# mcmilk/7-Zip-zstd

Measured on NVIDIA H100. Metric: zstd-L3 encode+decode throughput, higher is better.
Workload: dtype u8

## Files before the change

### 7-zip-zstd_b200/csrc/zstd_enc_entropy.cu

```cuda
#include "b2z_device.cuh"
#include "b2z_kernels.h"

namespace b2z {

__device__ const uint32_t d_LL_base[36] = { 0,1,2,3,4,5,6,7,8,9,10,11,12,13,14,15,
    16,18,20,22,24,28,32,40,48,64,0x80,0x100,0x200,0x400,0x800,0x1000,0x2000,0x4000,0x8000,0x10000 };
__device__ const uint8_t d_LL_bits[36] = { 0,0,0,0,0,0,0,0,0,0,0,0,0,0,0,0,
    1,1,1,1,2,2,3,3,4,6,7,8,9,10,11,12,13,14,15,16 };
__device__ const uint32_t d_ML_base[53] = { 3,4,5,6,7,8,9,10,11,12,13,14,15,16,17,18,
    19,20,21,22,23,24,25,26,27,28,29,30,31,32,33,34,
    35,37,39,41,43,47,51,59,67,83,99,0x83,0x103,0x203,0x403,0x803,0x1003,0x2003,0x4003,0x8003,0x10003 };
__device__ const uint8_t d_ML_bits[53] = { 0,0,0,0,0,0,0,0,0,0,0,0,0,0,0,0,
    0,0,0,0,0,0,0,0,0,0,0,0,0,0,0,0,
    1,1,1,1,2,2,3,3,4,4,5,7,8,9,10,11,12,13,14,15,16 };
__device__ const int16_t d_LL_defNorm[36] = { 4,3,2,2,2,2,2,2,2,2,2,2,2,1,1,1,
    2,2,2,2,2,2,2,2,2,3,2,1,1,1,1,1,-1,-1,-1,-1 };
__device__ const int16_t d_ML_defNorm[53] = { 1,4,3,2,2,2,2,2,2,1,1,1,1,1,1,1,
    1,1,1,1,1,1,1,1,1,1,1,1,1,1,1,1,
    1,1,1,1,1,1,1,1,1,1,1,1,1,1,-1,-1,-1,-1,-1,-1,-1 };
__device__ const int16_t d_OF_defNorm[29] = { 1,1,1,1,1,1,2,2,2,1,1,1,1,1,1,1,
    1,1,1,1,1,1,1,1,-1,-1,-1,-1,-1 };
__device__ const uint8_t d_log2frac[32] = { 0, 11, 22, 33, 43, 53, 63, 72, 82, 91, 100, 108, 116, 125, 132, 140,
    148, 155, 162, 169, 176, 182, 189, 195, 201, 207, 213, 219, 225, 230, 236, 241 };

__device__ __forceinline__ uint32_t ll_code(uint32_t ll) {
    if (ll < 16) return ll;
    if (ll < 24) return 16 + ((ll - 16) >> 1);
    if (ll < 32) return 20 + ((ll - 24) >> 2);
    if (ll < 48) return 22 + ((ll - 32) >> 3);
    if (ll < 64) return 24;
    return highbit32(ll) + 19;
}
__device__ __forceinline__ uint32_t ml_code(uint32_t m) {
    if (m < 32) return m;
    if (m < 40) return 32 + ((m - 32) >> 1);
    if (m < 48) return 36 + ((m - 40) >> 2);
    if (m < 64) return 38 + ((m - 48) >> 3);
    if (m < 96) return 40 + ((m - 64) >> 4);
    if (m < 128) return 42;
    return highbit32(m) + 36;
}

__device__ __forceinline__ uint32_t warp_sum(uint32_t v) {
    for (int d = 16; d; d >>= 1) v += __shfl_xor_sync(B2Z_FULL, v, d);
    return v;
}
__device__ __forceinline__ uint32_t warp_max(uint32_t v) {
    for (int d = 16; d; d >>= 1) { const uint32_t o = __shfl_xor_sync(B2Z_FULL, v, d); v = o > v ? o : v; }
    return v;
}

struct FseCT {
    uint16_t state[512];
    int32_t  dfs[64];
    uint32_t dnb[64];
    uint32_t log;
};

#define STAGE_WORDS 384
#define STAGE_FLUSH_BITS (STAGE_WORDS * 32 - 3072)

struct WarpWS {
    uint32_t hist[256];
    uint16_t hufCode[256];
    uint8_t  hufLen[256];
    union {
        struct { uint32_t w[512]; uint16_t parent[512]; uint8_t order[256]; uint8_t depth[512]; uint32_t key[256]; } hb;
        struct { FseCT ct[3]; } fse;
    } u;
    uint8_t  spread[512];
    int16_t  norm[64];
    uint16_t cumul[66];
    uint16_t cpos[66];
    uint32_t rk[16], rstart[16], rnext[16];
    uint32_t wcnt[16];
    uint32_t stage[STAGE_WORDS];
};

#define ENT_ST_OF 512u
#define ENT_ST_ML 768u
#define ENT_ST_N  1280u
#define ENT_SY_OF 36u
#define ENT_SY_ML 68u
#define ENT_SY_N  121u
struct EntTables {
    uint16_t state[ENT_ST_N];
    uint2    sym[ENT_SY_N];
    uint32_t pad[2];
};
struct EntRec {
    uint32_t run;
    uint32_t bodyHead;
    uint32_t logs;
    uint32_t pad0;
    uint16_t fin[4];
    uint32_t pad1[2];
    EntTables tab;
};
static_assert(sizeof(EntTables) % 16 == 0 && sizeof(EntRec) % 16 == 0 && offsetof(EntRec, tab) % 16 == 0, "EntRec is copied in 16-byte units");
#define ENT_SCRATCH_STRIDE ((size_t)sizeof(EntRec) + (size_t)B2Z_MAXSEQ * 4u)
static_assert(sizeof(EntRec) + (size_t)B2Z_MAXSEQ * 4u <= (size_t)B2Z_BLOCK * 4u, "stage E scratch must fit the block's candidate words");

struct BitW {
    uint8_t* p; uint64_t acc; uint32_t nb;
    __device__ __forceinline__ void init(uint8_t* q) { p = q; acc = 0; nb = 0; }
    __device__ __forceinline__ void add(uint32_t v, uint32_t n) {
        acc |= (uint64_t)(v & (n >= 32 ? 0xFFFFFFFFu : ((1u << n) - 1u))) << nb; nb += n;
        while (nb >= 8) { *p++ = (uint8_t)acc; acc >>= 8; nb -= 8; }
    }
    __device__ __forceinline__ uint8_t* close() { add(1, 1); if (nb) { *p++ = (uint8_t)acc; acc = 0; nb = 0; } return p; }
    __device__ __forceinline__ uint8_t* flush_partial() { if (nb) { *p++ = (uint8_t)acc; acc = 0; nb = 0; } return p; }
};

__device__ void fse_build_ctable(WarpWS* ws, FseCT* ct, const int16_t* norm, uint32_t maxSym, uint32_t log, uint32_t lane) {
    const uint32_t size = 1u << log, mask = size - 1u, step = (size >> 1) + (size >> 3) + 3u, lt = (1u << lane) - 1u;
    uint16_t* cumul = ws->cumul; uint16_t* cpos = ws->cpos; uint8_t* spread = ws->spread;
    uint32_t cu = 0, cp = 0, nLow = 0;
    for (uint32_t s0 = 0; s0 <= maxSym; s0 += 32) {
        const uint32_t s = s0 + lane;
        const int n = s <= maxSym ? norm[s] : 0;
        uint32_t tc, tp;
        const uint32_t ec = warp_excl_scan(n == -1 ? 1u : (n > 0 ? (uint32_t)n : 0u), lane, &tc);
        const uint32_t ep = warp_excl_scan(n > 0 ? (uint32_t)n : 0u, lane, &tp);
        const uint32_t low = __ballot_sync(B2Z_FULL, n == -1);
// ... 200 lines not shown
    maxW = warp_max(maxW);
    if (lane < 16) ws->wcnt[lane] = 0;
    __syncwarp();
    uint32_t fseSize = 0;
    if (nw > 1) {
        for (uint32_t s = lane; s < nw; s += 32) atomicAdd(&ws->wcnt[wt[s]], 1u);
        __syncwarp();
        const uint32_t maxCnt = warp_max(lane <= maxW ? ws->wcnt[lane] : 0u);
        if (maxCnt != nw && maxCnt > 1) {
            uint32_t log = 6;
            const uint32_t minBits = highbit32(nw) + 1u, symBits = highbit32(maxW + 1u) + 2u;
            const uint32_t lo = minBits < symBits ? minBits : symBits;
            const uint32_t want = highbit32(nw - 1u) >= 2u ? highbit32(nw - 1u) - 2u : 0u;
            if (want < log) log = want;
            if (log < lo) log = lo;
            if (log < 5) log = 5;
            if (log > 6) log = 6;
            int16_t* norm = ws->norm;
            fse_normalize(norm, log, ws->wcnt, nw, maxW, lane);
            uint8_t* tmp = dst + 1;
            uint32_t hs = 0;
            if (lane == 0) hs = fse_write_ncount(tmp, norm, maxW, log);
            hs = __shfl_sync(B2Z_FULL, hs, 0);
            FseCT* ct = reinterpret_cast<FseCT*>(ws->u.hb.w);
            fse_build_ctable(ws, ct, norm, maxW, log, lane);
            if (lane == 0) {
                BitW b; b.init(tmp + hs);
                uint32_t i = nw, s1, s2, nb, bits;
                if (nw & 1u) { s1 = fse_init_state(ct, wt[--i]); s2 = fse_init_state(ct, wt[--i]);
                               bits = fse_encode(ct, &s1, wt[--i], &nb); b.add(bits, nb); }
                else { s2 = fse_init_state(ct, wt[--i]); s1 = fse_init_state(ct, wt[--i]); }
                while (i > 0) {
                    bits = fse_encode(ct, &s2, wt[--i], &nb); b.add(bits, nb);
                    bits = fse_encode(ct, &s1, wt[--i], &nb); b.add(bits, nb);
                }
                b.add(s2, log); b.add(s1, log);
                fseSize = (uint32_t)(b.close() - tmp);
            }
            fseSize = __shfl_sync(B2Z_FULL, fseSize, 0);
        }
    }
    const uint32_t rawSize = (nw + 1u) / 2u;
    if (fseSize && fseSize < 128u && (fseSize < rawSize || nw > 128u)) { if (lane == 0) dst[0] = (uint8_t)fseSize; return 1u + fseSize; }
    if (nw > 128u || nw == 0u) return 0;
    if (lane == 0) dst[0] = (uint8_t)(127u + nw);
    for (uint32_t i = 2u * lane; i < nw; i += 64) dst[1 + i / 2] = (uint8_t)((wt[i] << 4) | (i + 1 < nw ? wt[i + 1] : 0));
    return 1u + rawSize;
}
static_assert(sizeof(FseCT) <= sizeof(uint32_t) * 512, "weights FseCT must fit in hb.w");

struct Stager {
    uint32_t* stage; uint8_t* out; uint32_t bits;
    __device__ __forceinline__ void init(uint32_t* s, uint8_t* o, uint32_t lane) {
        stage = s; out = o; bits = 0;
        for (uint32_t i = lane; i < STAGE_WORDS; i += 32) stage[i] = 0;
        __syncwarp();
    }
    __device__ __forceinline__ void put(uint32_t off, uint64_t lo, uint32_t hi, uint32_t nb) {
        if (!nb) return;
        const uint32_t wi = off >> 5, sh = off & 31u;
        const uint32_t w0 = (uint32_t)lo, w1 = (uint32_t)(lo >> 32);
        atomicOr(&stage[wi], w0 << sh);
        const uint32_t end = sh + nb;
        if (end > 32) atomicOr(&stage[wi + 1], sh ? (uint32_t)((((uint64_t)w1 << 32) | w0) >> (32 - sh)) : w1);
        if (end > 64) atomicOr(&stage[wi + 2], sh ? (uint32_t)((((uint64_t)hi << 32) | w1) >> (32 - sh)) : hi);
        if (end > 96) atomicOr(&stage[wi + 3], sh ? (hi >> (32 - sh)) : 0u);
    }
    __device__ __forceinline__ void flush(uint32_t lane, bool force) {
        __syncwarp();
        const uint32_t nbytes = force ? (bits + 7u) >> 3 : bits >> 3;
        const uint8_t* sb = reinterpret_cast<const uint8_t*>(stage);
        for (uint32_t i = lane; i < nbytes; i += 32) out[i] = sb[i];
        const uint32_t rem = force ? 0u : (bits & 7u);
        const uint32_t carry = rem ? sb[nbytes] : 0u;
        __syncwarp();
        for (uint32_t i = lane; i < STAGE_WORDS; i += 32) stage[i] = (i == 0) ? carry : 0u;
        __syncwarp();
        out += nbytes; bits = rem;
    }
};

__device__ uint32_t huf_encode_stream(WarpWS* ws, Stager& st, const uint8_t* __restrict__ lit, uint32_t a, uint32_t b, uint32_t lane) {
    uint8_t* start = st.out;
    for (uint32_t hi = b; hi > a;) {
        const uint32_t cnt = (hi - a) < 128u ? (hi - a) : 128u;
        uint64_t code = 0; uint32_t nb = 0;
#pragma unroll
        for (uint32_t j = 0; j < 4; j++) {
            const uint32_t k = lane * 4u + j;
            if (k < cnt) { const uint32_t s = lit[hi - 1u - k]; code |= (uint64_t)ws->hufCode[s] << nb; nb += ws->hufLen[s]; }
        }
        uint32_t total; const uint32_t off = warp_excl_scan(nb, lane, &total);
        st.put(st.bits + off, code, 0, nb);
        st.bits += total; hi -= cnt;
        if (st.bits > STAGE_FLUSH_BITS) st.flush(lane, false);
    }
    if (lane == 0) st.put(st.bits, 1, 0, 1);
    st.bits += 1;
    st.flush(lane, true);
    return (uint32_t)(st.out - start);
}

__device__ __forceinline__ void warp_copy(uint8_t* dst, const uint8_t* __restrict__ src, uint32_t n, uint32_t lane) {
    for (uint32_t i = lane; i < n; i += 32) dst[i] = src[i];
}

__device__ uint32_t choose_seq_table(WarpWS* ws, FseCT* ct, uint8_t* dst, const uint32_t* count, uint32_t nbSeq, uint32_t maxSymAll,
                                     uint32_t maxLog, const int16_t* defNorm, uint32_t defMaxSym, uint32_t defLog, uint32_t* mode, uint32_t lane) {
    uint32_t maxSym = 0, present = 0, big = 0;
    for (uint32_t s = lane; s <= maxSymAll; s += 32) if (count[s]) { maxSym = s; present++; if (count[s] > big) big = count[s]; }
    maxSym = warp_max(maxSym); present = warp_sum(present); big = warp_max(big);
    if (big == nbSeq && !(nbSeq <= 2 && maxSym <= defMaxSym)) {
        for (uint32_t s = lane; s < 64; s += 32) { ct->dnb[s] = 0; ct->dfs[s] = 0; }
        if (lane < 2) ct->state[lane] = 0;
        if (lane == 0) { ct->log = 0; dst[0] = (uint8_t)maxSym; }
        __syncwarp();
        *mode = 1; return 1;
    }
    int16_t* norm = ws->norm;
    uint64_t costDef = ~0ull;
    if (maxSym <= defMaxSym) {
        for (uint32_t s = lane; s <= defMaxSym; s += 32) norm[s] = defNorm[s];
        __syncwarp();
        costDef = fse_cost_fx8(count, norm, maxSym, defLog, lane);
        __syncwarp();
    }
    const uint32_t hbN = highbit32(nbSeq > 1 ? nbSeq - 1u : 1u);
    uint32_t log = hbN >= 2 ? hbN - 2u : 0u;
    const uint32_t minA = highbit32(nbSeq) + 1u, minB = highbit32(maxSym ? maxSym : 1u) + 2u, lo = minA < minB ? minA : minB;
    if (log > maxLog) log = maxLog;
    if (log < lo) log = lo;
    if (log < 5) log = 5;
    if (log > maxLog) log = maxLog;
    while ((1u << log) < present) log++;
    fse_normalize(norm, log, count, nbSeq, maxSym, lane);
    uint32_t hs = 0;
    if (lane == 0) hs = fse_write_ncount(dst, norm, maxSym, log);
    hs = __shfl_sync(B2Z_FULL, hs, 0);
    const uint64_t costFse = fse_cost_fx8(count, norm, maxSym, log, lane) + ((uint64_t)hs << 11);
    __syncwarp();
    if (costDef <= costFse || big == nbSeq) {
        for (uint32_t s = lane; s <= defMaxSym; s += 32) norm[s] = defNorm[s];
        __syncwarp();
        fse_build_ctable(ws, ct, norm, defMaxSym, defLog, lane); *mode = 0; return 0;
    }
    fse_build_ctable(ws, ct, norm, maxSym, log, lane); *mode = 2; return hs;
}

struct BlockGeom { uint32_t blkSize, last; size_t litOff; };
__device__ __forceinline__ BlockGeom block_geom(const EncGeom& g, uint64_t srcSize, uint32_t blk) {
    const uint32_t blocksPerFrame = 1u << (g.frameLog - 17u);
    const uint64_t frame = blk / blocksPerFrame; const uint32_t bif = blk % blocksPerFrame;
    const uint64_t f0 = frame << g.frameLog;
    const uint64_t fn = enc_frame_bytes(g, srcSize, frame);
    const uint64_t b0 = (uint64_t)bif << 17;
    BlockGeom r;
    r.blkSize = (uint32_t)((fn - b0) < B2Z_BLOCK ? (fn - b0) : B2Z_BLOCK);
    r.last = (b0 + r.blkSize == fn) ? 1u : 0u;
    r.litOff = (size_t)(f0 + b0);
    return r;
}
__device__ __forceinline__ void put_hdr3(uint8_t* out, uint32_t h) { out[0] = (uint8_t)h; out[1] = (uint8_t)(h >> 8); out[2] = (uint8_t)(h >> 16); }

__device__ uint32_t finish_block(uint8_t* out, const uint8_t* __restrict__ bsrc, uint32_t blkSize, uint32_t last, uint32_t bodySize, bool overCap, uint32_t lane) {
    if (!overCap && bodySize < blkSize) {
        if (lane == 0) put_hdr3(out, last | (2u << 1) | (bodySize << 3));
        return 3 + bodySize;
    }
    __syncwarp();
    if (lane == 0) put_hdr3(out, last | (blkSize << 3));
    warp_copy(out + 3, bsrc, blkSize, lane);
    return 3 + blkSize;
}

__global__ void __launch_bounds__(B2Z_ENT_WARPS * 32)
zstd_enc_tables_kernel(const uint8_t* __restrict__ src, uint64_t srcSize, EncGeom g,
                       const uint64_t* __restrict__ seqs, const uint32_t* __restrict__ nseqArr,
                       const uint8_t* __restrict__ lits, const uint32_t* __restrict__ nlitArr,
                       uint8_t* __restrict__ slots, uint32_t* __restrict__ slotSize, uint8_t* __restrict__ scratch, uint32_t nBlocks) {
    __shared__ WarpWS wsAll[B2Z_ENT_WARPS];
    const uint32_t lane = threadIdx.x & 31u, wib = threadIdx.x >> 5;
    WarpWS* ws = &wsAll[wib];
    for (uint32_t blk = blockIdx.x * B2Z_ENT_WARPS + wib; blk < nBlocks; blk += gridDim.x * B2Z_ENT_WARPS) {
        const BlockGeom bg = block_geom(g, srcSize, blk);
        const uint32_t blkSize = bg.blkSize, last = bg.last;
        const uint8_t* bsrc = src + bg.litOff;
        const uint8_t* lit = lits + bg.litOff;
        const uint64_t* sq = seqs + (size_t)blk * B2Z_MAXSEQ;
        const uint32_t nbSeq = nseqArr[blk], nlit = nlitArr[blk];
        uint8_t* out = slots + (size_t)blk * B2Z_SLOT;
        uint8_t* body = out + 3;
        EntRec* rec = reinterpret_cast<EntRec*>(scratch + (size_t)blk * ENT_SCRATCH_STRIDE);

        bool rle = false;
        if (blkSize > 1 && nbSeq == 1 && nlit == 1) {
            const uint64_t s0 = sq[0];
            rle = B2Z_SEQ_LL(s0) == 1 && B2Z_SEQ_ML(s0) == blkSize - 1u && B2Z_SEQ_OFFBASE(s0) == 4u;
        }
        if (rle) {
            if (lane == 0) { put_hdr3(out, last | (1u << 1) | (blkSize << 3)); out[3] = bsrc[0]; slotSize[blk] = 4; rec->run = 0; }
            continue;
        }

        for (uint32_t i = lane; i < 256; i += 32) ws->hist[i] = 0;
        __syncwarp();
        for (uint32_t i = lane * 4; i < nlit; i += 128) {
            const uint32_t v = *reinterpret_cast<const uint32_t*>(lit + i);
            const uint32_t k = nlit - i;
            atomicAdd(&ws->hist[v & 255u], 1u);
            if (k > 1) atomicAdd(&ws->hist[(v >> 8) & 255u], 1u);
            if (k > 2) atomicAdd(&ws->hist[(v >> 16) & 255u], 1u);
            if (k > 3) atomicAdd(&ws->hist[v >> 24], 1u);
        }
        __syncwarp();
        uint32_t ns = 0;
        for (uint32_t i = lane; i < 256; i += 32) ns += ws->hist[i] != 0;
        ns = warp_sum(ns);

        const uint32_t rawHdr = nlit < 32 ? 1u : (nlit < 4096 ? 2u : 3u);
        uint32_t litSecSize = 0;
        bool litDone = false;
        if (nlit >= B2Z_LIT_RLE_MIN && ns == 1) {
            if (lane == 0) {
                if (rawHdr == 1) body[0] = (uint8_t)(1u | (nlit << 3));
                else if (rawHdr == 2) { const uint32_t h = 1u | (1u << 2) | (nlit << 4); body[0] = (uint8_t)h; body[1] = (uint8_t)(h >> 8); }
                else put_hdr3(body, 1u | (3u << 2) | (nlit << 4));
                body[rawHdr] = lit[0];
            }
            litSecSize = rawHdr + 1; litDone = true;
        }
        if (!litDone && nlit >= B2Z_LIT_HUF_MIN && ns >= 2) {
            const bool four = nlit >= 256;
            const uint32_t lh = nlit < 1024 ? 3u : (nlit < 16384 ? 4u : 5u);
            uint32_t maxSym; const uint32_t maxBits = huf_build(ws, lane, &maxSym);
            const uint32_t ts = huf_write_table(ws, body + lh, maxBits, maxSym, lane);
            __syncwarp();
            uint32_t T = 0;
            for (uint32_t i = lane; i < 256; i += 32) T += ws->hist[i] * ws->hufLen[i];
            T = warp_sum(T);
            const uint32_t est = ts + (four ? 6u : 0u) + ((T + 7u) >> 3) + (four ? 4u : 1u);
            if (ts && lh + est < rawHdr + nlit) {
                uint8_t* p = body + lh + ts;
                Stager st;
                uint32_t bodySz;
                if (!four) { st.init(ws->stage, p, lane); bodySz = huf_encode_stream(ws, st, lit, 0, nlit, lane); }
                else {
                    const uint32_t seg = (nlit + 3u) / 4u;
                    st.init(ws->stage, p + 6, lane);
                    const uint32_t s1 = huf_encode_stream(ws, st, lit, 0, seg, lane);
                    const uint32_t s2 = huf_encode_stream(ws, st, lit, seg, 2 * seg, lane);
                    const uint32_t s3 = huf_encode_stream(ws, st, lit, 2 * seg, 3 * seg, lane);
                    const uint32_t s4 = huf_encode_stream(ws, st, lit, 3 * seg, nlit, lane);
                    if (lane == 0) { p[0] = (uint8_t)s1; p[1] = (uint8_t)(s1 >> 8); p[2] = (uint8_t)s2; p[3] = (uint8_t)(s2 >> 8); p[4] = (uint8_t)s3; p[5] = (uint8_t)(s3 >> 8); }
                    bodySz = 6 + s1 + s2 + s3 + s4;
                }
                const uint32_t csize = ts + bodySz;
                if (lane == 0) {
                    const uint32_t sf = !four ? 0u : (lh == 3 ? 1u : (lh == 4 ? 2u : 3u));
                    if (lh == 3) put_hdr3(body, 2u | (sf << 2) | (nlit << 4) | (csize << 14));
                    else if (lh == 4) { const uint32_t h = 2u | (sf << 2) | (nlit << 4) | (csize << 18); body[0] = (uint8_t)h; body[1] = (uint8_t)(h >> 8); body[2] = (uint8_t)(h >> 16); body[3] = (uint8_t)(h >> 24); }
                    else { const uint64_t h = 2ull | (sf << 2) | ((uint64_t)nlit << 4) | ((uint64_t)csize << 22);
                           body[0] = (uint8_t)h; body[1] = (uint8_t)(h >> 8); body[2] = (uint8_t)(h >> 16); body[3] = (uint8_t)(h >> 24); body[4] = (uint8_t)(h >> 32); }
                }
                litSecSize = lh + csize; litDone = true;
            }
        }
        if (!litDone) {
            if (lane == 0) {
                if (rawHdr == 1) body[0] = (uint8_t)(nlit << 3);
                else if (rawHdr == 2) { const uint32_t h = (1u << 2) | (nlit << 4); body[0] = (uint8_t)h; body[1] = (uint8_t)(h >> 8); }
                else put_hdr3(body, (3u << 2) | (nlit << 4));
            }
            warp_copy(body + rawHdr, lit, nlit, lane);
            litSecSize = rawHdr + nlit;
        }
        __syncwarp();

        uint8_t* sp = body + litSecSize;
        uint32_t seqSecSize;
        bool overCap = false;
        {
            uint32_t hdr;
            if (nbSeq < 128) { if (lane == 0) sp[0] = (uint8_t)nbSeq; hdr = 1; }
            else if (nbSeq < 0x7F00) { if (lane == 0) { sp[0] = (uint8_t)((nbSeq >> 8) + 128u); sp[1] = (uint8_t)nbSeq; } hdr = 2; }
            else { if (lane == 0) { sp[0] = 255; sp[1] = (uint8_t)(nbSeq - 0x7F00u); sp[2] = (uint8_t)((nbSeq - 0x7F00u) >> 8); } hdr = 3; }
            seqSecSize = hdr;
        }
        if (nbSeq) {
            uint32_t* cLL = ws->hist; uint32_t* cOF = ws->hist + 64; uint32_t* cML = ws->hist + 128;
            for (uint32_t i = lane; i < 192; i += 32) ws->hist[i] = 0;
            __syncwarp();
            uint32_t extra = 0;
            for (uint32_t i0 = 0; i0 < nbSeq; i0 += 128) {
                uint64_t v[4];
#pragma unroll
                for (uint32_t m = 0; m < 4; m++) { const uint32_t i = i0 + 32u * m + lane; v[m] = i < nbSeq ? sq[i] : 0ull; }
#pragma unroll
                for (uint32_t m = 0; m < 4; m++) {
                    const uint64_t s = v[m];
                    if (!s) continue;
                    const uint32_t cl = ll_code(B2Z_SEQ_LL(s)), cm = ml_code(B2Z_SEQ_ML(s) - 3u), co = highbit32(B2Z_SEQ_OFFBASE(s));
                    atomicAdd(&cLL[cl], 1u); atomicAdd(&cML[cm], 1u); atomicAdd(&cOF[co], 1u);
                    extra += d_LL_bits[cl] + d_ML_bits[cm] + co;
                }
            }
            extra = warp_sum(extra);
            __syncwarp();
            FseCT* ctL = &ws->u.fse.ct[0]; FseCT* ctO = &ws->u.fse.ct[1]; FseCT* ctM = &ws->u.fse.ct[2];
            uint8_t* tp = sp + seqSecSize + 1;
            uint32_t mL, mO, mM;
            tp += choose_seq_table(ws, ctL, tp, cLL, nbSeq, 35, 9, d_LL_defNorm, 35, 6, &mL, lane);
            tp += choose_seq_table(ws, ctO, tp, cOF, nbSeq, 31, 8, d_OF_defNorm, 28, 5, &mO, lane);
            tp += choose_seq_table(ws, ctM, tp, cML, nbSeq, 52, 9, d_ML_defNorm, 52, 6, &mM, lane);
            if (lane == 0) sp[seqSecSize] = (uint8_t)((mL << 6) | (mO << 4) | (mM << 2));
            seqSecSize += 1 + (uint32_t)(tp - (sp + seqSecSize + 1));
            const uint64_t upper = (uint64_t)nbSeq * (ctL->log + ctO->log + ctM->log) + 1ull + extra;
            overCap = (uint64_t)litSecSize + seqSecSize + ((upper + 7ull) >> 3) > B2Z_BODY_CAP;
            if (!overCap) {
                for (uint32_t i = lane; i < ENT_ST_N; i += 32)
                    rec->tab.state[i] = i < ENT_ST_OF ? ctL->state[i] : (i < ENT_ST_ML ? ctO->state[i - ENT_ST_OF] : ctM->state[i - ENT_ST_ML]);
                for (uint32_t i = lane; i < ENT_SY_N; i += 32) {
                    const FseCT* ct = i < ENT_SY_OF ? ctL : (i < ENT_SY_ML ? ctO : ctM);
                    const uint32_t s = i < ENT_SY_OF ? i : (i < ENT_SY_ML ? i - ENT_SY_OF : i - ENT_SY_ML);
                    rec->tab.sym[i] = make_uint2(ct->dnb[s], (uint32_t)ct->dfs[s]);
                }
                if (lane == 0) { rec->run = 1; rec->bodyHead = litSecSize + seqSecSize; rec->logs = ctL->log | (ctO->log << 8) | (ctM->log << 16); }
                __syncwarp();
                continue;
            }
        }
        __syncwarp();
        const uint32_t outSize = finish_block(out, bsrc, blkSize, last, litSecSize + seqSecSize, overCap, lane);
        if (lane == 0) { slotSize[blk] = outSize; rec->run = 0; }
        __syncwarp();
    }
}

#define ENT_CHAIN_BLOCKS 10
#define ENT_CHAIN_SEQS   48
#define ENT_CHAIN_LOADS  (ENT_CHAIN_BLOCKS * ENT_CHAIN_SEQS / 32)
__global__ void __launch_bounds__(32)
zstd_enc_chains_kernel(const uint64_t* __restrict__ seqs, const uint32_t* __restrict__ nseqArr, uint8_t* __restrict__ scratch, uint32_t nBlocks) {
    __shared__ EntTables tabs[ENT_CHAIN_BLOCKS];
    __shared__ uint32_t codes[ENT_CHAIN_BLOCKS][ENT_CHAIN_SEQS];
    __shared__ uint32_t nsq[ENT_CHAIN_BLOCKS];
    const uint32_t lane = threadIdx.x, b = lane / 3u, t = lane - 3u * b;
    for (uint32_t blk0 = blockIdx.x * ENT_CHAIN_BLOCKS; blk0 < nBlocks; blk0 += gridDim.x * ENT_CHAIN_BLOCKS) {
        const uint32_t nb = nBlocks - blk0 < ENT_CHAIN_BLOCKS ? nBlocks - blk0 : ENT_CHAIN_BLOCKS;
        for (uint32_t j = 0; j < nb; j++) {
            const EntRec* r = reinterpret_cast<const EntRec*>(scratch + (size_t)(blk0 + j) * ENT_SCRATCH_STRIDE);
            if (!r->run) continue;
            const uint4* s4 = reinterpret_cast<const uint4*>(&r->tab);
            uint4* d4 = reinterpret_cast<uint4*>(&tabs[j]);
            for (uint32_t i = lane; i < sizeof(EntTables) / 16u; i += 32) d4[i] = s4[i];
        }
        if (lane < ENT_CHAIN_BLOCKS)
            nsq[lane] = lane < nb && reinterpret_cast<const EntRec*>(scratch + (size_t)(blk0 + lane) * ENT_SCRATCH_STRIDE)->run ? nseqArr[blk0 + lane] : 0u;
        __syncwarp();
        const uint32_t blk = blk0 + b;
        const bool mine = b < nb;
        const uint32_t n = mine ? nsq[b] : 0u;
        EntRec* rec = reinterpret_cast<EntRec*>(scratch + (size_t)(mine ? blk : blk0) * ENT_SCRATCH_STRIDE);
        uint32_t* words = reinterpret_cast<uint32_t*>(scratch + (size_t)blk * ENT_SCRATCH_STRIDE + sizeof(EntRec));
        const uint16_t* stT = tabs[mine ? b : 0].state + (t == 0 ? 0u : (t == 1 ? ENT_ST_OF : ENT_ST_ML));
        const uint2* syT = tabs[mine ? b : 0].sym + (t == 0 ? 0u : (t == 1 ? ENT_SY_OF : ENT_SY_ML));
        const uint32_t nMax = warp_max(n);
        uint32_t state = 0;
        for (uint32_t k0 = 0; k0 < nMax; k0 += ENT_CHAIN_SEQS) {
            uint64_t v[ENT_CHAIN_LOADS];
#pragma unroll
            for (uint32_t m = 0; m < ENT_CHAIN_LOADS; m++) {
                const uint32_t j = lane + 32u * m, bj = j / ENT_CHAIN_SEQS, k = k0 + j % ENT_CHAIN_SEQS, nj = nsq[bj];
                v[m] = k < nj ? seqs[(size_t)(blk0 + bj) * B2Z_MAXSEQ + (nj - 1u - k)] : 0ull;
            }
#pragma unroll
            for (uint32_t m = 0; m < ENT_CHAIN_LOADS; m++) {
                const uint32_t j = lane + 32u * m;
                const uint64_t s = v[m];
                codes[j / ENT_CHAIN_SEQS][j % ENT_CHAIN_SEQS] = s ? ll_code(B2Z_SEQ_LL(s)) | (highbit32(B2Z_SEQ_OFFBASE(s)) << 8) | (ml_code(B2Z_SEQ_ML(s) - 3u) << 16) : 0u;
            }
            __syncwarp();
            const uint32_t kEnd = nMax - k0 < ENT_CHAIN_SEQS ? nMax - k0 : ENT_CHAIN_SEQS;
            for (uint32_t kk = 0; kk < kEnd; kk++) {
                const uint32_t k = k0 + kk;
                const bool act = k < n;
                uint32_t bits = 0, nbits = 0;
                if (act) {
                    const uint32_t sym = (codes[b][kk] >> (8u * t)) & 255u;
                    const uint2 e = syT[sym];
                    if (k == 0) {
                        const uint32_t nb0 = (e.x + (1u << 15)) >> 16;
                        state = stT[(((nb0 << 16) - e.x) >> nb0) + e.y];
                    } else {
                        nbits = (state + e.x) >> 16; bits = state & ((1u << nbits) - 1u);
                        state = stT[(state >> nbits) + e.y];
                    }
                }
                const uint32_t oB = __shfl_down_sync(B2Z_FULL, bits, 1), oN = __shfl_down_sync(B2Z_FULL, nbits, 1);
                const uint32_t mB = __shfl_down_sync(B2Z_FULL, bits, 2), mN = __shfl_down_sync(B2Z_FULL, nbits, 2);
                if (act && t == 0) words[n - 1u - k] = oB | (mB << oN) | (bits << (oN + mN)) | ((oN + mN + nbits) << 26);
            }
            __syncwarp();
        }
        if (n) rec->fin[t] = (uint16_t)state;
        __syncwarp();
    }
}

__global__ void __launch_bounds__(B2Z_ENT_WARPS * 32)
zstd_enc_seqbits_kernel(const uint8_t* __restrict__ src, uint64_t srcSize, EncGeom g,
                        const uint64_t* __restrict__ seqs, const uint32_t* __restrict__ nseqArr,
                        uint8_t* __restrict__ slots, uint32_t* __restrict__ slotSize, const uint8_t* __restrict__ scratch, uint32_t nBlocks) {
    __shared__ uint32_t stageAll[B2Z_ENT_WARPS][STAGE_WORDS];
    const uint32_t lane = threadIdx.x & 31u, wib = threadIdx.x >> 5;
    for (uint32_t blk = blockIdx.x * B2Z_ENT_WARPS + wib; blk < nBlocks; blk += gridDim.x * B2Z_ENT_WARPS) {
        const EntRec* rec = reinterpret_cast<const EntRec*>(scratch + (size_t)blk * ENT_SCRATCH_STRIDE);
        if (!rec->run) continue;
        const uint32_t* words = reinterpret_cast<const uint32_t*>(scratch + (size_t)blk * ENT_SCRATCH_STRIDE + sizeof(EntRec));
        const BlockGeom bg = block_geom(g, srcSize, blk);
        const uint64_t* sq = seqs + (size_t)blk * B2Z_MAXSEQ;
        const uint32_t nbSeq = nseqArr[blk], bodyHead = rec->bodyHead, logs = rec->logs;
        const uint32_t logL = logs & 255u, logO = (logs >> 8) & 255u, logM = logs >> 16;
        uint8_t* out = slots + (size_t)blk * B2Z_SLOT;
        Stager st; st.init(stageAll[wib], out + 3 + bodyHead, lane);
        uint8_t* bsStart = st.out;
        for (uint32_t hi = nbSeq; hi > 0;) {
            const uint32_t cnt = hi < 32u ? hi : 32u;
            uint64_t lo = 0; uint32_t hiw = 0, nb = 0;
            if (lane < cnt) {
                const uint32_t i = hi - 1u - lane;
                const uint64_t s = sq[i]; const uint32_t w = words[i];
                const uint32_t llv = B2Z_SEQ_LL(s), mlv = B2Z_SEQ_ML(s), obv = B2Z_SEQ_OFFBASE(s);
                const uint32_t cl = ll_code(llv), cm = ml_code(mlv - 3u), co = highbit32(obv);
                lo = w & 0x3FFFFFFu; nb = w >> 26;
                const uint32_t lb = d_LL_bits[cl], mb = d_ML_bits[cm];
                lo |= (uint64_t)(llv - d_LL_base[cl]) << nb; nb += lb;
                lo |= (uint64_t)(mlv - d_ML_base[cm]) << nb; nb += mb;
                const uint32_t ox = obv - (1u << co);
                if (nb + co <= 64) { lo |= (co ? ((uint64_t)ox << nb) : 0ull); }
                else { lo |= (uint64_t)ox << nb; hiw = (uint32_t)((uint64_t)ox >> (64u - nb)); }
                nb += co;
            }
            uint32_t total; const uint32_t off = warp_excl_scan(nb, lane, &total);
            st.put(st.bits + off, lo, hiw, nb);
            st.bits += total; hi -= cnt;
            if (st.bits > STAGE_FLUSH_BITS) st.flush(lane, false);
        }
        if (lane == 0) {
            uint32_t o = st.bits;
            st.put(o, rec->fin[2] & ((1u << logM) - 1u), 0, logM); o += logM;
            st.put(o, rec->fin[1] & ((1u << logO) - 1u), 0, logO); o += logO;
            st.put(o, rec->fin[0] & ((1u << logL) - 1u), 0, logL); o += logL;
            st.put(o, 1, 0, 1);
        }
        st.bits += logM + logO + logL + 1u;
        st.flush(lane, true);
        const uint32_t bodySize = bodyHead + (uint32_t)(st.out - bsStart);
        const uint32_t outSize = finish_block(out, src + bg.litOff, bg.blkSize, bg.last, bodySize, false, lane);
        if (lane == 0) slotSize[blk] = outSize;
        __syncwarp();
    }
}

#ifndef B2Z_CUEMU
void launch_zstd_enc_entropy(const uint8_t* src, uint64_t srcSize, const EncGeom& g,
                             const uint64_t* seqs, const uint32_t* nseq, const uint8_t* lits, const uint32_t* nlit,
                             uint8_t* slots, uint32_t* slotSize, uint8_t* scratch, uint32_t nBlocks, uint32_t smCount, cudaStream_t st) {
    if (!nBlocks) return;
    uint32_t grid = (nBlocks + B2Z_ENT_WARPS - 1) / B2Z_ENT_WARPS;
    const uint32_t cap = smCount * 16u;
    if (grid > cap) grid = cap;
    zstd_enc_tables_kernel<<<grid, B2Z_ENT_WARPS * 32, 0, st>>>(src, srcSize, g, seqs, nseq, lits, nlit, slots, slotSize, scratch, nBlocks);
    zstd_enc_chains_kernel<<<(nBlocks + ENT_CHAIN_BLOCKS - 1) / ENT_CHAIN_BLOCKS, 32, 0, st>>>(seqs, nseq, scratch, nBlocks);
    zstd_enc_seqbits_kernel<<<grid, B2Z_ENT_WARPS * 32, 0, st>>>(src, srcSize, g, seqs, nseq, slots, slotSize, scratch, nBlocks);
}
#else
inline void zstd_enc_entropy_kernel(const uint8_t* src, uint64_t srcSize, EncGeom g, const uint64_t* seqs, const uint32_t* nseq,
                                    const uint8_t* lits, const uint32_t* nlit, uint8_t* slots, uint32_t* slotSize, uint32_t nBlocks) {
    if (blockIdx.x != 0 || threadIdx.x != 0 || !nBlocks) return;
    cuemu::Block* const outer = cuemu::blk();
    std::vector<uint8_t> buf((size_t)nBlocks * ENT_SCRATCH_STRIDE + 16, 0xCD);
    uint8_t* const scratch = buf.data() + ((16u - ((uintptr_t)buf.data() & 15u)) & 15u);
    const dim3 grid((nBlocks + B2Z_ENT_WARPS - 1) / B2Z_ENT_WARPS), block(B2Z_ENT_WARPS * 32);
    uint64_t c = cuemu::launch(grid, block, 0, [&] { zstd_enc_tables_kernel(src, srcSize, g, seqs, nseq, lits, nlit, slots, slotSize, scratch, nBlocks); });
    c += cuemu::launch(dim3((nBlocks + ENT_CHAIN_BLOCKS - 1) / ENT_CHAIN_BLOCKS), dim3(32), 0, [&] { zstd_enc_chains_kernel(seqs, nseq, scratch, nBlocks); });
    c += cuemu::launch(grid, block, 0, [&] { zstd_enc_seqbits_kernel(src, srcSize, g, seqs, nseq, slots, slotSize, scratch, nBlocks); });
    cuemu::blk() = outer;
    outer->collectives += c;
}
#endif

}
```

Baseline: 33010.

## Restructure FSE chain kernel to one lane per block using precomputed codes

The tables kernel now writes per-sequence LL/OF/ML codes into scratch and aggregates histogram atomics with warp match. The chains kernel then assigns one lane per entropy block, running all three FSE state chains serially over those precomputed codes with vectorized prefetched loads, instead of three lanes per block with per-step shuffles. It also adds lookup tables for length codes, uint4-vectorized literal histograms, and prefetching in Huffman encoding, plus optional clock instrumentation. The chains kernel now uses dynamic shared memory for more blocks per warp, and cudaFuncSetAttribute is called on every launch, which adds a little host overhead.

```diff
diff --git a/7-zip-zstd_b200/csrc/zstd_enc_entropy.cu b/7-zip-zstd_b200/csrc/zstd_enc_entropy.cu
--- a/7-zip-zstd_b200/csrc/zstd_enc_entropy.cu
+++ b/7-zip-zstd_b200/csrc/zstd_enc_entropy.cu
@@ -23,23 +23,27 @@
 __device__ const uint8_t d_log2frac[32] = { 0, 11, 22, 33, 43, 53, 63, 72, 82, 91, 100, 108, 116, 125, 132, 140,
     148, 155, 162, 169, 176, 182, 189, 195, 201, 207, 213, 219, 225, 230, 236, 241 };
 
-__device__ __forceinline__ uint32_t ll_code(uint32_t ll) {
-    if (ll < 16) return ll;
-    if (ll < 24) return 16 + ((ll - 16) >> 1);
-    if (ll < 32) return 20 + ((ll - 24) >> 2);
-    if (ll < 48) return 22 + ((ll - 32) >> 3);
-    if (ll < 64) return 24;
-    return highbit32(ll) + 19;
-}
-__device__ __forceinline__ uint32_t ml_code(uint32_t m) {
-    if (m < 32) return m;
-    if (m < 40) return 32 + ((m - 32) >> 1);
-    if (m < 48) return 36 + ((m - 40) >> 2);
-    if (m < 64) return 38 + ((m - 48) >> 3);
-    if (m < 96) return 40 + ((m - 64) >> 4);
-    if (m < 128) return 42;
-    return highbit32(m) + 36;
-}
+__device__ const uint8_t d_LL_code[64] = { 0,1,2,3,4,5,6,7,8,9,10,11,12,13,14,15,16,16,17,17,18,18,19,19,20,20,20,20,21,21,21,21,
+    22,22,22,22,22,22,22,22,23,23,23,23,23,23,23,23,24,24,24,24,24,24,24,24,24,24,24,24,24,24,24,24 };
+__device__ const uint8_t d_ML_code[128] = { 0,1,2,3,4,5,6,7,8,9,10,11,12,13,14,15,16,17,18,19,20,21,22,23,24,25,26,27,28,29,30,31,
+    32,32,33,33,34,34,35,35,36,36,36,36,37,37,37,37,38,38,38,38,38,38,38,38,39,39,39,39,39,39,39,39,
+    40,40,40,40,40,40,40,40,40,40,40,40,40,40,40,40,41,41,41,41,41,41,41,41,41,41,41,41,41,41,41,41,
+    42,42,42,42,42,42,42,42,42,42,42,42,42,42,42,42,42,42,42,42,42,42,42,42,42,42,42,42,42,42,42,42 };
+__device__ __forceinline__ uint32_t ll_code(uint32_t ll) { return ll < 64 ? (uint32_t)d_LL_code[ll] : highbit32(ll) + 19u; }
+__device__ __forceinline__ uint32_t ml_code(uint32_t m) { return m < 128 ? (uint32_t)d_ML_code[m] : highbit32(m) + 36u; }
+
+enum { E1C_LITHIST, E1C_HUF, E1C_LITSTREAMS, E1C_SEQPASS, E1C_TABLES, E1C_HANDOFF, E1C_N };
+enum { E2C_STAGE, E2C_LOAD, E2C_STEP, E2C_STORE, E2C_N };
+#if defined(B2Z_E_CLOCKS) && !defined(B2Z_CUEMU)
+__device__ unsigned long long e_clocks[E1C_N + E2C_N];
+#define E_CLOCKS_START(n) unsigned long long ec_[n] = {}; long long ecLast_ = clock64()
+#define E_TICK(ph) do { const long long now_ = clock64(); ec_[ph] += (unsigned long long)(now_ - ecLast_); ecLast_ = now_; } while (0)
+#define E_CLOCKS_FLUSH(base, n) do { if (lane == 0) for (int p_ = 0; p_ < (n); p_++) atomicAdd(&e_clocks[(base) + p_], ec_[p_]); } while (0)
+#else
+#define E_CLOCKS_START(n) do { } while (0)
+#define E_TICK(ph) do { } while (0)
+#define E_CLOCKS_FLUSH(base, n) do { } while (0)
+#endif
 
 __device__ __forceinline__ uint32_t warp_sum(uint32_t v) {
     for (int d = 16; d; d >>= 1) v += __shfl_xor_sync(B2Z_FULL, v, d);
@@ -406,14 +410,22 @@
 
 __device__ uint32_t huf_encode_stream(WarpWS* ws, Stager& st, const uint8_t* __restrict__ lit, uint32_t a, uint32_t b, uint32_t lane) {
     uint8_t* start = st.out;
+    uint32_t cur[4];
+#pragma unroll
+    for (uint32_t j = 0; j < 4; j++) { const uint32_t k = lane * 4u + j; cur[j] = k < b - a ? lit[b - 1u - k] : 0u; }
     for (uint32_t hi = b; hi > a;) {
-        const uint32_t cnt = (hi - a) < 128u ? (hi - a) : 128u;
+        const uint32_t cnt = (hi - a) < 128u ? (hi - a) : 128u, hn = hi - cnt;
+        uint32_t nxt[4];
+#pragma unroll
+        for (uint32_t j = 0; j < 4; j++) { const uint32_t k = lane * 4u + j; nxt[j] = k < hn - a ? lit[hn - 1u - k] : 0u; }
         uint64_t code = 0; uint32_t nb = 0;
 #pragma unroll
         for (uint32_t j = 0; j < 4; j++) {
             const uint32_t k = lane * 4u + j;
-            if (k < cnt) { const uint32_t s = lit[hi - 1u - k]; code |= (uint64_t)ws->hufCode[s] << nb; nb += ws->hufLen[s]; }
-        }
+            if (k < cnt) { const uint32_t s = cur[j]; code |= (uint64_t)ws->hufCode[s] << nb; nb += ws->hufLen[s]; }
+        }
+#pragma unroll
+        for (uint32_t j = 0; j < 4; j++) cur[j] = nxt[j];
         uint32_t total; const uint32_t off = warp_excl_scan(nb, lane, &total);
         st.put(st.bits + off, code, 0, nb);
         st.bits += total; hi -= cnt;
@@ -505,6 +517,7 @@
     __shared__ WarpWS wsAll[B2Z_ENT_WARPS];
     const uint32_t lane = threadIdx.x & 31u, wib = threadIdx.x >> 5;
     WarpWS* ws = &wsAll[wib];
+    E_CLOCKS_START(E1C_N);
     for (uint32_t blk = blockIdx.x * B2Z_ENT_WARPS + wib; blk < nBlocks; blk += gridDim.x * B2Z_ENT_WARPS) {
         const BlockGeom bg = block_geom(g, srcSize, blk);
         const uint32_t blkSize = bg.blkSize, last = bg.last;
@@ -528,18 +541,28 @@
 
         for (uint32_t i = lane; i < 256; i += 32) ws->hist[i] = 0;
         __syncwarp();
-        for (uint32_t i = lane * 4; i < nlit; i += 128) {
-            const uint32_t v = *reinterpret_cast<const uint32_t*>(lit + i);
-            const uint32_t k = nlit - i;
-            atomicAdd(&ws->hist[v & 255u], 1u);
-            if (k > 1) atomicAdd(&ws->hist[(v >> 8) & 255u], 1u);
-            if (k > 2) atomicAdd(&ws->hist[(v >> 16) & 255u], 1u);
-            if (k > 3) atomicAdd(&ws->hist[v >> 24], 1u);
+        {
+            const uint4* lit4 = reinterpret_cast<const uint4*>(lit);
+            const uint32_t nv = (nlit + 15u) >> 4;
+            uint4 cur = lane < nv ? lit4[lane] : make_uint4(0, 0, 0, 0);
+            for (uint32_t v0 = 0; v0 < nv; v0 += 32) {
+                const uint32_t vi = v0 + lane;
+                const uint4 nxt = vi + 32u < nv ? lit4[vi + 32u] : make_uint4(0, 0, 0, 0);
+                if (vi < nv) {
+                    const uint32_t w[4] = { cur.x, cur.y, cur.z, cur.w };
+                    const uint32_t k = nlit - 16u * vi;
+#pragma unroll
+                    for (uint32_t j = 0; j < 16; j++)
+                        if (j < k) atomicAdd(&ws->hist[(w[j >> 2] >> (8u * (j & 3u))) & 255u], 1u);
+                }
+                cur = nxt;
+            }
         }
         __syncwarp();
         uint32_t ns = 0;
         for (uint32_t i = lane; i < 256; i += 32) ns += ws->hist[i] != 0;
         ns = warp_sum(ns);
+        E_TICK(E1C_LITHIST);
 
         const uint32_t rawHdr = nlit < 32 ? 1u : (nlit < 4096 ? 2u : 3u);
         uint32_t litSecSize = 0;
@@ -562,6 +585,7 @@
             uint32_t T = 0;
             for (uint32_t i = lane; i < 256; i += 32) T += ws->hist[i] * ws->hufLen[i];
             T = warp_sum(T);
+            E_TICK(E1C_HUF);
             const uint32_t est = ts + (four ? 6u : 0u) + ((T + 7u) >> 3) + (four ? 4u : 1u);
             if (ts && lh + est < rawHdr + nlit) {
                 uint8_t* p = body + lh + ts;
@@ -599,6 +623,7 @@
             litSecSize = rawHdr + nlit;
         }
         __syncwarp();
+        E_TICK(E1C_LITSTREAMS);
 
         uint8_t* sp = body + litSecSize;
         uint32_t seqSecSize;
@@ -614,22 +639,35 @@
             uint32_t* cLL = ws->hist; uint32_t* cOF = ws->hist + 64; uint32_t* cML = ws->hist + 128;
             for (uint32_t i = lane; i < 192; i += 32) ws->hist[i] = 0;
             __syncwarp();
+            uint32_t* codeOut = reinterpret_cast<uint32_t*>(scratch + (size_t)blk * ENT_SCRATCH_STRIDE + sizeof(EntRec));
             uint32_t extra = 0;
+            uint64_t v[4];
+#pragma unroll
+            for (uint32_t m = 0; m < 4; m++) { const uint32_t i = 32u * m + lane; v[m] = i < nbSeq ? sq[i] : 0ull; }
             for (uint32_t i0 = 0; i0 < nbSeq; i0 += 128) {
-                uint64_t v[4];
-#pragma unroll
-                for (uint32_t m = 0; m < 4; m++) { const uint32_t i = i0 + 32u * m + lane; v[m] = i < nbSeq ? sq[i] : 0ull; }
+                uint64_t nx[4];
+#pragma unroll
+                for (uint32_t m = 0; m < 4; m++) { const uint32_t i = i0 + 128u + 32u * m + lane; nx[m] = i < nbSeq ? sq[i] : 0ull; }
 #pragma unroll
                 for (uint32_t m = 0; m < 4; m++) {
                     const uint64_t s = v[m];
-                    if (!s) continue;
-                    const uint32_t cl = ll_code(B2Z_SEQ_LL(s)), cm = ml_code(B2Z_SEQ_ML(s) - 3u), co = highbit32(B2Z_SEQ_OFFBASE(s));
-                    atomicAdd(&cLL[cl], 1u); atomicAdd(&cML[cm], 1u); atomicAdd(&cOF[co], 1u);
-                    extra += d_LL_bits[cl] + d_ML_bits[cm] + co;
+                    const bool ok = s != 0;
+                    const uint32_t cl = ok ? ll_code(B2Z_SEQ_LL(s)) : 255u, cm = ok ? ml_code(B2Z_SEQ_ML(s) - 3u) : 255u, co = ok ? highbit32(B2Z_SEQ_OFFBASE(s)) : 255u;
+                    const uint32_t gl = __match_any_sync(B2Z_FULL, cl), gm = __match_any_sync(B2Z_FULL, cm), go = __match_any_sync(B2Z_FULL, co);
+                    if (ok) {
+                        codeOut[i0 + 32u * m + lane] = cl | (co << 8) | (cm << 16);
+                        if (lane == (uint32_t)__ffs((int)gl) - 1u) atomicAdd(&cLL[cl], (uint32_t)__popc(gl));
+                        if (lane == (uint32_t)__ffs((int)gm) - 1u) atomicAdd(&cML[cm], (uint32_t)__popc(gm));
+                        if (lane == (uint32_t)__ffs((int)go) - 1u) atomicAdd(&cOF[co], (uint32_t)__popc(go));
+                        extra += d_LL_bits[cl] + d_ML_bits[cm] + co;
+                    }
                 }
+#pragma unroll
+                for (uint32_t m = 0; m < 4; m++) v[m] = nx[m];
             }
             extra = warp_sum(extra);
             __syncwarp();
+            E_TICK(E1C_SEQPASS);
             FseCT* ctL = &ws->u.fse.ct[0]; FseCT* ctO = &ws->u.fse.ct[1]; FseCT* ctM = &ws->u.fse.ct[2];
             uint8_t* tp = sp + seqSecSize + 1;
             uint32_t mL, mO, mM;
@@ -638,6 +676,7 @@
             tp += choose_seq_table(ws, ctM, tp, cML, nbSeq, 52, 9, d_ML_defNorm, 52, 6, &mM, lane);
             if (lane == 0) sp[seqSecSize] = (uint8_t)((mL << 6) | (mO << 4) | (mM << 2));
             seqSecSize += 1 + (uint32_t)(tp - (sp + seqSecSize + 1));
+            E_TICK(E1C_TABLES);
             const uint64_t upper = (uint64_t)nbSeq * (ctL->log + ctO->log + ctM->log) + 1ull + extra;
             overCap = (uint64_t)litSecSize + seqSecSize + ((upper + 7ull) >> 3) > B2Z_BODY_CAP;
             if (!overCap) {
@@ -650,6 +689,7 @@
                 }
                 if (lane == 0) { rec->run = 1; rec->bodyHead = litSecSize + seqSecSize; rec->logs = ctL->log | (ctO->log << 8) | (ctM->log << 16); }
                 __syncwarp();
+                E_TICK(E1C_HANDOFF);
                 continue;
             }
         }
@@ -657,78 +697,103 @@
         const uint32_t outSize = finish_block(out, bsrc, blkSize, last, litSecSize + seqSecSize, overCap, lane);
         if (lane == 0) { slotSize[blk] = outSize; rec->run = 0; }
         __syncwarp();
-    }
-}
-
-#define ENT_CHAIN_BLOCKS 10
-#define ENT_CHAIN_SEQS   48
-#define ENT_CHAIN_LOADS  (ENT_CHAIN_BLOCKS * ENT_CHAIN_SEQS / 32)
+        E_TICK(E1C_HANDOFF);
+    }
+    E_CLOCKS_FLUSH(0, E1C_N);
+}
+
+#define ENT_CHAIN_BLOCKS 16
+#define ENT_CHAIN_VECS   4
+#define ENT_CHAIN_SMEM   ((size_t)ENT_CHAIN_BLOCKS * sizeof(EntTables))
+__device__ __forceinline__ uint32_t fse_first_state(const uint16_t* stT, uint2 e) {
+    const uint32_t nb = (e.x + (1u << 15)) >> 16;
+    return stT[(((nb << 16) - e.x) >> nb) + e.y];
+}
+__device__ __forceinline__ uint32_t fse_step(const uint16_t* stT, uint2 e, uint32_t& state, uint32_t& nbits) {
+    nbits = (state + e.x) >> 16;
+    const uint32_t bits = state & ((1u << nbits) - 1u);
+    state = stT[(state >> nbits) + e.y];
+    return bits;
+}
 __global__ void __launch_bounds__(32)
-zstd_enc_chains_kernel(const uint64_t* __restrict__ seqs, const uint32_t* __restrict__ nseqArr, uint8_t* __restrict__ scratch, uint32_t nBlocks) {
-    __shared__ EntTables tabs[ENT_CHAIN_BLOCKS];
-    __shared__ uint32_t codes[ENT_CHAIN_BLOCKS][ENT_CHAIN_SEQS];
-    __shared__ uint32_t nsq[ENT_CHAIN_BLOCKS];
-    const uint32_t lane = threadIdx.x, b = lane / 3u, t = lane - 3u * b;
+zstd_enc_chains_kernel(const uint32_t* __restrict__ nseqArr, uint8_t* __restrict__ scratch, uint32_t nBlocks) {
+    B2Z_DYN_SMEM(EntTables, tabs);
+    const uint32_t lane = threadIdx.x;
+    E_CLOCKS_START(E2C_N);
     for (uint32_t blk0 = blockIdx.x * ENT_CHAIN_BLOCKS; blk0 < nBlocks; blk0 += gridDim.x * ENT_CHAIN_BLOCKS) {
-        const uint32_t nb = nBlocks - blk0 < ENT_CHAIN_BLOCKS ? nBlocks - blk0 : ENT_CHAIN_BLOCKS;
-        for (uint32_t j = 0; j < nb; j++) {
-            const EntRec* r = reinterpret_cast<const EntRec*>(scratch + (size_t)(blk0 + j) * ENT_SCRATCH_STRIDE);
-            if (!r->run) continue;
-            const uint4* s4 = reinterpret_cast<const uint4*>(&r->tab);
+        const uint32_t blk = blk0 + lane;
+        EntRec* rec = reinterpret_cast<EntRec*>(scratch + (size_t)blk * ENT_SCRATCH_STRIDE);
+        const bool mine = lane < ENT_CHAIN_BLOCKS && blk < nBlocks && rec->run;
+        const uint32_t n = mine ? nseqArr[blk] : 0u;
+        for (uint32_t run = __ballot_sync(B2Z_FULL, mine); run; run &= run - 1u) {
+            const uint32_t j = (uint32_t)__ffs((int)run) - 1u;
+            const uint4* s4 = reinterpret_cast<const uint4*>(&reinterpret_cast<const EntRec*>(scratch + (size_t)(blk0 + j) * ENT_SCRATCH_STRIDE)->tab);
             uint4* d4 = reinterpret_cast<uint4*>(&tabs[j]);
             for (uint32_t i = lane; i < sizeof(EntTables) / 16u; i += 32) d4[i] = s4[i];
         }
-        if (lane < ENT_CHAIN_BLOCKS)
-            nsq[lane] = lane < nb && reinterpret_cast<const EntRec*>(scratch + (size_t)(blk0 + lane) * ENT_SCRATCH_STRIDE)->run ? nseqArr[blk0 + lane] : 0u;
-        __syncwarp();
-        const uint32_t blk = blk0 + b;
-        const bool mine = b < nb;
-        const uint32_t n = mine ? nsq[b] : 0u;
-        EntRec* rec = reinterpret_cast<EntRec*>(scratch + (size_t)(mine ? blk : blk0) * ENT_SCRATCH_STRIDE);
-        uint32_t* words = reinterpret_cast<uint32_t*>(scratch + (size_t)blk * ENT_SCRATCH_STRIDE + sizeof(EntRec));
-        const uint16_t* stT = tabs[mine ? b : 0].state + (t == 0 ? 0u : (t == 1 ? ENT_ST_OF : ENT_ST_ML));
-        const uint2* syT = tabs[mine ? b : 0].sym + (t == 0 ? 0u : (t == 1 ? ENT_SY_OF : ENT_SY_ML));
-        const uint32_t nMax = warp_max(n);
-        uint32_t state = 0;
-        for (uint32_t k0 = 0; k0 < nMax; k0 += ENT_CHAIN_SEQS) {
-            uint64_t v[ENT_CHAIN_LOADS];
-#pragma unroll
-            for (uint32_t m = 0; m < ENT_CHAIN_LOADS; m++) {
-                const uint32_t j = lane + 32u * m, bj = j / ENT_CHAIN_SEQS, k = k0 + j % ENT_CHAIN_SEQS, nj = nsq[bj];
-                v[m] = k < nj ? seqs[(size_t)(blk0 + bj) * B2Z_MAXSEQ + (nj - 1u - k)] : 0ull;
-            }
-#pragma unroll
-            for (uint32_t m = 0; m < ENT_CHAIN_LOADS; m++) {
-                const uint32_t j = lane + 32u * m;
-                const uint64_t s = v[m];
-                codes[j / ENT_CHAIN_SEQS][j % ENT_CHAIN_SEQS] = s ? ll_code(B2Z_SEQ_LL(s)) | (highbit32(B2Z_SEQ_OFFBASE(s)) << 8) | (ml_code(B2Z_SEQ_ML(s) - 3u) << 16) : 0u;
-            }
-            __syncwarp();
-            const uint32_t kEnd = nMax - k0 < ENT_CHAIN_SEQS ? nMax - k0 : ENT_CHAIN_SEQS;
-            for (uint32_t kk = 0; kk < kEnd; kk++) {
-                const uint32_t k = k0 + kk;
-                const bool act = k < n;
-                uint32_t bits = 0, nbits = 0;
-                if (act) {
-                    const uint32_t sym = (codes[b][kk] >> (8u * t)) & 255u;
-                    const uint2 e = syT[sym];
-                    if (k == 0) {
-                        const uint32_t nb0 = (e.x + (1u << 15)) >> 16;
-                        state = stT[(((nb0 << 16) - e.x) >> nb0) + e.y];
-                    } else {
-                        nbits = (state + e.x) >> 16; bits = state & ((1u << nbits) - 1u);
-                        state = stT[(state >> nbits) + e.y];
+        __syncwarp();
+        E_TICK(E2C_STAGE);
+        const EntTables* tb = &tabs[mine ? lane : 0u];
+        const uint16_t* stL = tb->state; const uint16_t* stO = tb->state + ENT_ST_OF; const uint16_t* stM = tb->state + ENT_ST_ML;
+        const uint2* sy = tb->sym;
+        uint4* w4 = reinterpret_cast<uint4*>(scratch + (size_t)(mine ? blk : blk0) * ENT_SCRATCH_STRIDE + sizeof(EntRec));
+        const int32_t nV = (int32_t)((n + 3u) >> 2), last = (int32_t)n - 1;
+        const uint32_t rounds = warp_max(((uint32_t)nV + ENT_CHAIN_VECS - 1u) / ENT_CHAIN_VECS);
+        uint4 cur[ENT_CHAIN_VECS];
+#pragma unroll
+        for (int32_t m = 0; m < ENT_CHAIN_VECS; m++) { const int32_t q = nV - 1 - m; cur[m] = q >= 0 ? w4[q] : make_uint4(0, 0, 0, 0); }
+        uint32_t sL = 0, sO = 0, sM = 0;
+        if (n) {
+            const uint32_t e = (uint32_t)last & 3u;
+            const uint32_t c = e == 0 ? cur[0].x : (e == 1 ? cur[0].y : (e == 2 ? cur[0].z : cur[0].w));
+            sL = fse_first_state(stL, sy[c & 255u]);
+            sO = fse_first_state(stO, sy[ENT_SY_OF + ((c >> 8) & 255u)]);
+            sM = fse_first_state(stM, sy[ENT_SY_ML + (c >> 16)]);
+        }
+        E_TICK(E2C_LOAD);
+        for (uint32_t r = 0; r < rounds; r++) {
+            const int32_t q0 = nV - 1 - (int32_t)(r * ENT_CHAIN_VECS);
+            uint4 nxt[ENT_CHAIN_VECS];
+#pragma unroll
+            for (int32_t m = 0; m < ENT_CHAIN_VECS; m++) {
+                const int32_t q = q0 - ENT_CHAIN_VECS - m;
+                nxt[m] = q >= 0 ? w4[q] : make_uint4(0, 0, 0, 0);
+            }
+            E_TICK(E2C_LOAD);
+#pragma unroll
+            for (int32_t m = 0; m < ENT_CHAIN_VECS; m++) {
+                const int32_t q = q0 - m;
+                if (q < 0) continue;
+                uint32_t w[4] = { cur[m].x, cur[m].y, cur[m].z, cur[m].w };
+#pragma unroll
+                for (int32_t e = 3; e >= 0; e--) {
+                    const int32_t i = 4 * q + e;
+                    if (i < last) {
+                        const uint32_t c = w[e];
+                        const uint2 eL = sy[c & 255u], eO = sy[ENT_SY_OF + ((c >> 8) & 255u)], eM = sy[ENT_SY_ML + (c >> 16)];
+                        uint32_t nL, nO, nM;
+                        const uint32_t bO = fse_step(stO, eO, sO, nO), bM = fse_step(stM, eM, sM, nM), bL = fse_step(stL, eL, sL, nL);
+                        w[e] = bO | (bM << nO) | (bL << (nO + nM)) | ((nO + nM + nL) << 26);
+                    } else if (i == last) {
+                        w[e] = 0;
                     }
                 }
-                const uint32_t oB = __shfl_down_sync(B2Z_FULL, bits, 1), oN = __shfl_down_sync(B2Z_FULL, nbits, 1);
-                const uint32_t mB = __shfl_down_sync(B2Z_FULL, bits, 2), mN = __shfl_down_sync(B2Z_FULL, nbits, 2);
-                if (act && t == 0) words[n - 1u - k] = oB | (mB << oN) | (bits << (oN + mN)) | ((oN + mN + nbits) << 26);
-            }
-            __syncwarp();
-        }
-        if (n) rec->fin[t] = (uint16_t)state;
-        __syncwarp();
-    }
+                cur[m] = make_uint4(w[0], w[1], w[2], w[3]);
+            }
+            E_TICK(E2C_STEP);
+#pragma unroll
+            for (int32_t m = 0; m < ENT_CHAIN_VECS; m++) {
+                const int32_t q = q0 - m;
+                if (q >= 0) w4[q] = cur[m];
+                cur[m] = nxt[m];
+            }
+            E_TICK(E2C_STORE);
+        }
+        if (n) { rec->fin[0] = (uint16_t)sL; rec->fin[1] = (uint16_t)sO; rec->fin[2] = (uint16_t)sM; }
+        __syncwarp();
+        E_TICK(E2C_STORE);
+    }
+    E_CLOCKS_FLUSH(E1C_N, E2C_N);
 }
 
 __global__ void __launch_bounds__(B2Z_ENT_WARPS * 32)
@@ -787,6 +852,14 @@
 }
 
 #ifndef B2Z_CUEMU
+#ifdef B2Z_E_CLOCKS
+extern "C" int b200z_e_clocks(unsigned long long* out) {
+    static const unsigned long long zero[E1C_N + E2C_N] = {};
+    cudaError_t e = cudaMemcpyFromSymbol(out, e_clocks, sizeof(e_clocks));
+    if (e == cudaSuccess) e = cudaMemcpyToSymbol(e_clocks, zero, sizeof(e_clocks));
+    return (int)e;
+}
+#endif
 void launch_zstd_enc_entropy(const uint8_t* src, uint64_t srcSize, const EncGeom& g,
                              const uint64_t* seqs, const uint32_t* nseq, const uint8_t* lits, const uint32_t* nlit,
                              uint8_t* slots, uint32_t* slotSize, uint8_t* scratch, uint32_t nBlocks, uint32_t smCount, cudaStream_t st) {
@@ -795,7 +868,9 @@
     const uint32_t cap = smCount * 16u;
     if (grid > cap) grid = cap;
     zstd_enc_tables_kernel<<<grid, B2Z_ENT_WARPS * 32, 0, st>>>(src, srcSize, g, seqs, nseq, lits, nlit, slots, slotSize, scratch, nBlocks);
-    zstd_enc_chains_kernel<<<(nBlocks + ENT_CHAIN_BLOCKS - 1) / ENT_CHAIN_BLOCKS, 32, 0, st>>>(seqs, nseq, scratch, nBlocks);
+    cudaFuncSetAttribute(zstd_enc_chains_kernel, cudaFuncAttributeMaxDynamicSharedMemorySize, (int)ENT_CHAIN_SMEM);
+    cudaFuncSetAttribute(zstd_enc_chains_kernel, cudaFuncAttributePreferredSharedMemoryCarveout, 100);
+    zstd_enc_chains_kernel<<<(nBlocks + ENT_CHAIN_BLOCKS - 1) / ENT_CHAIN_BLOCKS, 32, ENT_CHAIN_SMEM, st>>>(nseq, scratch, nBlocks);
     zstd_enc_seqbits_kernel<<<grid, B2Z_ENT_WARPS * 32, 0, st>>>(src, srcSize, g, seqs, nseq, slots, slotSize, scratch, nBlocks);
 }
 #else
@@ -807,7 +882,7 @@
     uint8_t* const scratch = buf.data() + ((16u - ((uintptr_t)buf.data() & 15u)) & 15u);
     const dim3 grid((nBlocks + B2Z_ENT_WARPS - 1) / B2Z_ENT_WARPS), block(B2Z_ENT_WARPS * 32);
     uint64_t c = cuemu::launch(grid, block, 0, [&] { zstd_enc_tables_kernel(src, srcSize, g, seqs, nseq, lits, nlit, slots, slotSize, scratch, nBlocks); });
-    c += cuemu::launch(dim3((nBlocks + ENT_CHAIN_BLOCKS - 1) / ENT_CHAIN_BLOCKS), dim3(32), 0, [&] { zstd_enc_chains_kernel(seqs, nseq, scratch, nBlocks); });
+    c += cuemu::launch(dim3((nBlocks + ENT_CHAIN_BLOCKS - 1) / ENT_CHAIN_BLOCKS), dim3(32), ENT_CHAIN_SMEM, [&] { zstd_enc_chains_kernel(nseq, scratch, nBlocks); });
     c += cuemu::launch(grid, block, 0, [&] { zstd_enc_seqbits_kernel(src, srcSize, g, seqs, nseq, slots, slotSize, scratch, nBlocks); });
     cuemu::blk() = outer;
     outer->collectives += c;
```

After: 35350, median of 6. 7.1% higher.
